# IRFM/librir

Measured on AMD Instinct MI355X. Metric: IR frames/sec encode+decode, 640x512 uint16, higher is better.
Workload: dtype u16; 1 GPU; configs[1]: 1000-frame 640x512 uint16 stream (S1 noisy background, seed 1234+rank), lossless RIRB1 encode+decode, device-resident, GOP 50, per GPU; two launches per step: the encoder leaves the PACKED form (headers + position and length per segment + the payload without holes: encoded_footprint_bytes, in a buffer of half the raw size), the decoder reads it as it is; the compressed payload (17 % of; frames_per_gpu=1000, width=640, height=512, gop=50

## Files before the change

librir_amd/csrc/codec_kernels.hip:

```cpp
#include <hip/hip_runtime.h>
#include <algorithm>
#include <stdint.h>

#include "codec_format.h"
#include "filter_kernels.h"
#include "runtime.h"

namespace rir
{

	constexpr int FRAME_LOAD_AUX = 2;
	constexpr int FRAME_STORE_AUX = 2;
	constexpr int SPARSE_STORE_AUX = 0;
	constexpr int STREAM_LOAD_AUX = 0;

	typedef short short2v __attribute__((ext_vector_type(2)));
	typedef unsigned short ushort2v __attribute__((ext_vector_type(2)));

	__device__ __forceinline__ uint32_t pk_sub16(uint32_t a, uint32_t b)
	{
		return __builtin_bit_cast(uint32_t, __builtin_bit_cast(ushort2v, a) - __builtin_bit_cast(ushort2v, b));
	}
	__device__ __forceinline__ uint32_t pk_add16(uint32_t a, uint32_t b)
	{
// ... 539 lines not shown
	{
		__shared__ uint32_t wave_tot[4];
		__shared__ uint32_t carry_s;
		const int c = blockIdx.x, tid = threadIdx.x, lane = tid & 63, wv = tid >> 6;
		const uint32_t *in = seg_words + (int64_t)c * ntiles;
		uint32_t *off = tile_off + (int64_t)c * (ntiles + 1);
		if (tid == 0)
			carry_s = 0;
		__syncthreads();
		for (int base = 0; base < ntiles; base += 256)
		{
			const int i = base + tid;
			const uint32_t v = i < ntiles ? in[i] : 0u;
			const uint32_t inc = wave_scan_add(v, lane);
			if (lane == 63)
				wave_tot[wv] = inc;
			__syncthreads();
			uint32_t pre = carry_s;
			for (int k = 0; k < wv; ++k)
				pre += wave_tot[k];
			if (i < ntiles)
				off[i] = pre + inc - v;
			__syncthreads();
			if (tid == 255)
				carry_s = pre + inc;
			__syncthreads();
		}
		if (tid == 0)
		{
			off[ntiles] = carry_s;
			chunk_words[c] = carry_s;
		}
	}

	__global__ __launch_bounds__(256) void rirb1_compact(const uint64_t *__restrict__ sparse, const uint32_t *__restrict__ tile_off,
														const uint64_t *__restrict__ chunk_words, int ntiles, int nchunks, int gop,
														uint64_t *__restrict__ chunk_off, uint64_t *__restrict__ stream)
	{
		const int t = blockIdx.x, c = blockIdx.y, tid = threadIdx.x;
		const uint32_t *off = tile_off + (int64_t)c * (ntiles + 1);
		const uint32_t o0 = off[t], o1 = off[t + 1];
		uint64_t s = 0;
		for (int i = tid & 63; i < c; i += 64)
			s += chunk_words[i];
#pragma unroll
		for (int d = 32; d >= 1; d >>= 1)
			s += (uint64_t)__shfl_xor((long long)s, d, 64);
		if (t == 0 && tid == 0)
		{
			chunk_off[c] = s;
			if (c == nchunks - 1)
				chunk_off[nchunks] = s + chunk_words[c];
		}
		const uint32_t n = o1 - o0;
		const uint64_t *src = sparse + ((int64_t)c * ntiles + t) * RIRB1_SLOT_WORDS(gop);
		uint64_t *dst = stream + s + o0;
		uint32_t i = tid;
		for (; i + 768 < n; i += 1024)
		{
			const uint64_t v0 = __builtin_nontemporal_load(src + i);
			const uint64_t v1 = __builtin_nontemporal_load(src + i + 256);
			const uint64_t v2 = __builtin_nontemporal_load(src + i + 512);
			const uint64_t v3 = __builtin_nontemporal_load(src + i + 768);
			dst[i] = v0, dst[i + 256] = v1, dst[i + 512] = v2, dst[i + 768] = v3;
		}
		for (; i < n; i += 256)
			dst[i] = __builtin_nontemporal_load(src + i);
	}

#define RIR_LB_TAG (1ull << 63)
#define RIR_LB_TIMEOUT_TICKS 200000000ull
	constexpr int LB_SLEEP = 8;
#define RIR_NONE 0xffffffffu

	struct RecordWords
	{
		v2u32 va, vb;
		uint32_t ia, ib;
	};

	__device__ __forceinline__ uint64_t emit_words_narrow(const Px8 &r, uint32_t mode, uint32_t base, RecordWords &rw, uint32_t pos, const LaneConsts &lc,
														  const TransposeConsts &tc, uint32_t *words)
	{
		uint32_t x = (r.d[0] | (r.d[1] << 8)) | ((r.d[2] | (r.d[3] << 8)) << 4);
		x = transpose32(x, tc);
		const uint64_t nz64 = __ballot(x != 0);
		const uint32_t nz = (uint32_t)nz64 | (uint32_t)(nz64 >> 32);
		uint32_t M = nz | ((nz >> 1) & 0x77777777u);
		M |= (M >> 2) & 0x33333333u;
		uint32_t W = M - ((M >> 1) & 0x55555555u);
		W = (W & 0x33333333u) + ((W >> 2) & 0x33333333u);
		*words = (uint32_t)__builtin_popcount(M);
		auto sw = __builtin_amdgcn_permlane32_swap(x, x, false, false);
		rw.va.x = x, rw.va.y = sw[1];
		rw.ia = __builtin_amdgcn_inverse_ballot_w64((uint64_t)M) ? pos + (uint32_t)__builtin_popcount(M & lc.p_before) : RIR_NONE;
		rw.vb = rw.va, rw.ib = RIR_NONE;
		const uint32_t B = base | (mode << 16);
		const uint64_t hw = __ballot((int32_t)(W << lc.p_hshw) < 0) & 0x00E700E700E700E7ull;
		const uint64_t hb = __ballot((int32_t)(B << lc.p_hshb) < 0) & 0x3C003C003C00FC00ull;
		return hw | hb;
	}

	__device__ __forceinline__ uint64_t emit_words_wide(const Px8 &r, uint32_t mode, uint32_t base, RecordWords &rw, uint32_t pos, const LaneConsts &lc,
														const TransposeConsts &tc, uint32_t *words)
	{
		uint32_t alo = r.d[0], ahi = r.d[1], blo = r.d[2], bhi = r.d[3];
		transpose64x2(alo, ahi, blo, bhi, tc);
		const uint32_t wa = row_allmax((alo | ahi) != 0 ? lc.bitp1 : 0u);
		const uint32_t wb = row_allmax((blo | bhi) != 0 ? lc.bitp1 : 0u);
		const uint32_t ia = rows_inclusive_sum(wa), ib = rows_inclusive_sum(wb);
		const uint32_t tot_a = (uint32_t)__builtin_amdgcn_readlane((int)ia, 63);
		const uint32_t tot_b = (uint32_t)__builtin_amdgcn_readlane((int)ib, 63);
		rw.va.x = alo, rw.va.y = ahi, rw.vb.x = blo, rw.vb.y = bhi;
		rw.ia = lc.bit < wa ? pos + ia - wa + lc.bit : RIR_NONE;
		rw.ib = lc.bit < wb ? pos + tot_a + ib - wb + lc.bit : RIR_NONE;
		*words = tot_a + tot_b;
		const uint32_t nib = (base >> lc.sh4) & 15u;
		const uint32_t field = ((nib << 10) | (lc.row0 ? mode << 14 : 0u)) | ((wb << 5) | wa);
		return __ballot((field & lc.onehot) != 0);
	}

	struct Staging
	{
		uint64_t *lds;
		uint32_t cap;
		uint32_t lds_used;
		bool spilling;
		__amdgpu_buffer_rsrc_t spill;
		uint64_t *arena;
		unsigned long long *cursor;
		uint64_t arena_words;
		uint32_t need;
		uint64_t extent;
		uint32_t *error_word;
	};

	__device__ __noinline__ uint64_t staging_take_extent(unsigned long long *cursor, uint32_t need, uint64_t arena_words, uint32_t *error_word)
	{
		unsigned long long off = 0;
		if ((threadIdx.x & 63u) == 0)
			off = __hip_atomic_fetch_add(cursor, (unsigned long long)need, __ATOMIC_RELAXED, __HIP_MEMORY_SCOPE_AGENT);
		const uint32_t lo = (uint32_t)__builtin_amdgcn_readfirstlane((int)(uint32_t)off);
		const uint32_t hi = (uint32_t)__builtin_amdgcn_readfirstlane((int)(uint32_t)(off >> 32));
		off = ((unsigned long long)hi << 32) | lo;
		if (off + need > arena_words)
		{
			if ((threadIdx.x & 63u) == 0)
				__hip_atomic_fetch_or(error_word, 2u, __ATOMIC_RELAXED, __HIP_MEMORY_SCOPE_AGENT);
			return ~0ull;
		}
		return off;
	}

	__device__ __forceinline__ uint64_t emit_staged(const Px8 &r, uint32_t mode, uint32_t base, Staging &sg, uint32_t pos, const LaneConsts &lc,
													const TransposeConsts &tc, uint32_t *words)
	{
		const uint32_t any = (r.d[0] | r.d[1]) | (r.d[2] | r.d[3]);
		RecordWords rw;
		uint64_t h;
		if (__ballot((any & 0xfff0fff0u) != 0) == 0)
			h = emit_words_narrow(r, mode, base, rw, pos, lc, tc, words);
		else
			h = emit_words_wide(r, mode, base, rw, pos, lc, tc, words);
		if (!sg.spilling && pos + *words > sg.cap)
		{
			sg.spilling = true, sg.lds_used = pos;
			if (sg.arena)
			{
				const uint64_t ext = staging_take_extent(sg.cursor, sg.need, sg.arena_words, sg.error_word);
				sg.extent = ((uint64_t)(uint32_t)__builtin_amdgcn_readfirstlane((int)(uint32_t)(ext >> 32)) << 32) |
							(uint32_t)__builtin_amdgcn_readfirstlane((int)(uint32_t)ext);
				if (sg.extent != ~0ull)
					sg.spill = make_rsrc(sg.arena + sg.extent, sg.need * 8u);
			}
		}
		if (!sg.spilling)
		{
			if (rw.ia != RIR_NONE)
				sg.lds[rw.ia] = ((uint64_t)rw.va.y << 32) | rw.va.x;
			if (rw.ib != RIR_NONE)
				sg.lds[rw.ib] = ((uint64_t)rw.vb.y << 32) | rw.vb.x;
		}
		const uint32_t add = sg.spilling ? 0u - sg.lds_used * 8u : RIR_OOB;
		const uint32_t oa = rw.ia != RIR_NONE ? rw.ia * 8u + add : RIR_OOB;
		const uint32_t ob = rw.ib != RIR_NONE ? rw.ib * 8u + add : RIR_OOB;
		__builtin_amdgcn_raw_buffer_store_b64(rw.va, sg.spill, oa, 0, SPARSE_STORE_AUX);
		__builtin_amdgcn_raw_buffer_store_b64(rw.vb, sg.spill, ob, 0, SPARSE_STORE_AUX);
		return h;
	}

	template <bool FAST>
	__device__ __forceinline__ uint32_t encode_run(const uint16_t *__restrict__ frames, int64_t npx, int nload, int64_t frame_first, bool has_key,
												   int tile, int lane, uint64_t *__restrict__ hdr_first, Staging &sg)
	{
		const int64_t p0 = (int64_t)tile * RIRB1_TILE_PX + lane * 8;
		const TransposeConsts tc = make_transpose_consts(lane);
		const LaneConsts lc = make_lane_consts(lane);
		const uint32_t lane_off = (uint32_t)lane * 16u;
		const uint16_t *next_ptr = frames + frame_first * npx + (int64_t)tile * RIRB1_TILE_PX;
		int next_f = 0;
		auto load = [&](int f, v4u32 &dst) {
			if (FAST)
			{
				const Px8 p = buf_load8(next_ptr, next_f < nload ? lane_off : RIR_OOB);
				dst.x = p.d[0], dst.y = p.d[1], dst.z = p.d[2], dst.w = p.d[3];
				next_ptr += npx;
				next_f += 1;
			}
			else
			{
				const Px8 p = load8(frames, frame_first + min(f, nload - 1), npx, p0, false);
				dst.x = p.d[0], dst.y = p.d[1], dst.z = p.d[2], dst.w = p.d[3];
			}
		};
		auto as_px8 = [](const v4u32 &v) {
			Px8 p;
			p.d[0] = v.x, p.d[1] = v.y, p.d[2] = v.z, p.d[3] = v.w;
			return p;
		};
		uint32_t pos = 0;
		uint64_t hdr_reg = 0;
		v4u32 s0, s1, s2, s3;
		load(0, s0);
		load(1, s1);
		load(2, s2);
		load(3, s3);
		if (has_key)
		{
			const Px8 cur = as_px8(s0);
			const uint32_t base_raw = tile_base(cur, false);
			const uint32_t b2 = base_raw | (base_raw << 16);
			Px8 r_raw;
#pragma unroll
			for (int k = 0; k < 4; ++k)
				r_raw.d[k] = pk_sub16(cur.d[k], b2);
			const Px8 dl = left_delta(cur, lane);
			const uint32_t base_left = tile_base(dl, true);
			const uint32_t bl2 = base_left | (base_left << 16);
			Px8 r_left;
#pragma unroll
			for (int k = 0; k < 4; ++k)
				r_left.d[k] = pk_sub16(dl.d[k], bl2);
			const bool use_left = payload_words(r_left) < payload_words(r_raw);
			Px8 r_sel;
#pragma unroll
			for (int k = 0; k < 4; ++k)
				r_sel.d[k] = use_left ? r_left.d[k] : r_raw.d[k];
			uint32_t words;
			const uint32_t key_mode = use_left ? RIRB1_MODE_LEFT : RIRB1_MODE_RAW;
			const uint64_t h = emit_staged(r_sel, key_mode, use_left ? base_left : base_raw, sg, pos, lc, tc, &words);
			if (lane == 0)
				hdr_first[0] = h;
			pos += words;
		}
#define RIR_ENC2_STEP(F, CUR, PREV)                                                            \
	{                                                                                          \
		const int f = (F);                                                                     \
		Px8 d;                                                                                 \
		{                                                                                      \
			const Px8 c_ = as_px8(CUR), p_ = as_px8(PREV);                                     \
			_Pragma("unroll") for (int k = 0; k < 4; ++k) d.d[k] = pk_sub16(c_.d[k], p_.d[k]); \
		}                                                                                      \
		load(f + 3, PREV);                                                                     \
		const uint32_t base = tile_base(d, true);                                              \
		const uint32_t b2 = base | (base << 16);                                               \
		_Pragma("unroll") for (int k = 0; k < 4; ++k) d.d[k] = pk_sub16(d.d[k], b2);          \
		uint32_t words;                                                                        \
		const uint64_t h = emit_staged(d, RIRB1_MODE_TEMPORAL, base, sg, pos, lc, tc, &words); \
		if (lane == ((f - 1) & 63))                                                            \
			hdr_reg = h;                                                                       \
		pos += words;                                                                          \
	}
		int fb = 1;
		while (fb < nload)
		{
			const int g0 = fb, gend = min(fb + 64, nload);
			for (; fb + 3 < gend; fb += 4)
			{
				RIR_ENC2_STEP(fb, s1, s0)
				RIR_ENC2_STEP(fb + 1, s2, s1)
				RIR_ENC2_STEP(fb + 2, s3, s2)
				RIR_ENC2_STEP(fb + 3, s0, s3)
			}
			if (fb < gend)
			{
				RIR_ENC2_STEP(fb, s1, s0)
				if (fb + 1 < gend)
				{
					RIR_ENC2_STEP(fb + 1, s2, s1)
					if (fb + 2 < gend)
						RIR_ENC2_STEP(fb + 2, s3, s2)
				}
				fb = gend;
			}
			if (g0 + lane < gend)
				hdr_first[g0 + lane] = hdr_reg;
			hdr_reg = 0;
		}
#undef RIR_ENC2_STEP
		return pos;
	}

	__device__ __forceinline__ uint64_t wave_sum_u64(uint64_t v)
	{
#pragma unroll
		for (int d = 32; d >= 1; d >>= 1)
			v += (uint64_t)__shfl_xor((long long)v, d, 64);
		return v;
	}

	__device__ __noinline__ bool encode_lookback(const uint64_t *P, const uint64_t *gtotal, const uint64_t *gran, uint32_t *error_word, int c, int t,
												 int ntiles, int ngroups, int lane, uint64_t *A_out, uint64_t *P_out, uint64_t * )
	{
		const int g = t >> 6, e1 = t & 63, E = e1 + g + (c > 0 ? 1 : 0);
		uint64_t accA = 0, accP = 0;
		const uint64_t t_start = __builtin_amdgcn_s_memrealtime();
		for (int e0 = 0; e0 < E; e0 += 64)
		{
			const int e = e0 + lane;
			const bool valid = e < E;
			int kind = 2;
			const uint64_t *ptr = P + c;
			if (e < e1)
				kind = 0, ptr = gran + (int64_t)c * ntiles + ((int64_t)g << 6) + e;
			else if (e < e1 + g)
				kind = 1, ptr = gtotal + (int64_t)c * ngroups + (e - e1);
			uint64_t v = 0;
			bool done = !valid;
			for (uint32_t spins = 0;; ++spins)
			{
				if (!done)
				{
					v = __hip_atomic_load(ptr, __ATOMIC_RELAXED, __HIP_MEMORY_SCOPE_AGENT);
					done = (v >> 63) != 0;
				}
				if (__ballot(!done) == 0)
					break;
				if ((spins & 15u) == 15u)
				{
					const uint32_t err = __hip_atomic_load(error_word, __ATOMIC_RELAXED, __HIP_MEMORY_SCOPE_AGENT);
					if (err != 0 || __builtin_amdgcn_s_memrealtime() - t_start > RIR_LB_TIMEOUT_TICKS)
					{
						if (lane == 0)
							__hip_atomic_store(error_word, 1u, __ATOMIC_RELAXED, __HIP_MEMORY_SCOPE_AGENT);
						return false;
					}
				}
				__builtin_amdgcn_s_sleep(LB_SLEEP);
			}
			if (valid)
			{
				if (kind == 2)
					accP = v & ~RIR_LB_TAG;
				else
					accA += v & ~RIR_LB_TAG;
			}
		}
		*A_out = wave_sum_u64(accA);
		*P_out = wave_sum_u64(accP);
		return true;
	}

	__device__ __host__ __forceinline__ int enc_split(int w, int waves, int nf)
	{
		if (w <= 0)
			return 0;
		if (w >= waves)
			return nf;
		const int b = (w * (nf + 1) + waves / 2) / waves - 1;
		return b < 1 ? (nf < 1 ? nf : 1) : (b > nf ? nf : b);
	}

	__device__ __host__ __forceinline__ int64_t enc_ctrl_words64(int nchunks, int ntiles)
	{
		const int64_t ngroups = (ntiles + 63) / 64;
		return 8 * 16 + 16 + ((int64_t)nchunks + 1) + (int64_t)nchunks * ngroups + (((int64_t)nchunks * ntiles + 15) & ~(int64_t)15) +
			   (int64_t)nchunks * ngroups + nchunks + 16;
	}

	template <int WAVES>
	__attribute__((amdgpu_waves_per_eu(8, 8))) __global__ __launch_bounds__(WAVES * 64) void rirb1_encode_dense(
		const uint16_t *__restrict__ frames, int64_t npx, int ntiles, int nframes, int gop, int nchunks, uint64_t *__restrict__ hdr_table,
		uint32_t *__restrict__ tile_off, uint64_t *__restrict__ chunk_off, uint64_t *__restrict__ stream, uint64_t *__restrict__ ctrl,
		uint64_t *__restrict__ spill, int cap)
	{
		extern __shared__ __attribute__((aligned(16))) uint64_t enc_lds[];
		uint64_t *sh_base = enc_lds + (size_t)WAVES * cap;
		uint32_t *sh_u32 = reinterpret_cast<uint32_t *>(sh_base + 1);
		const int lane = threadIdx.x & 63;
		const int w = __builtin_amdgcn_readfirstlane((int)(threadIdx.x >> 6));
		const int ngroups = (ntiles + 63) >> 6;
		uint32_t *heads = reinterpret_cast<uint32_t *>(ctrl);
		uint32_t *error_word = reinterpret_cast<uint32_t *>(ctrl + 8 * 16);
		uint64_t *P = ctrl + 8 * 16 + 16;
		uint64_t *gtotal = P + nchunks + 1;
		uint64_t *gran = gtotal + (int64_t)nchunks * ngroups;
		uint64_t *gcount = gran + (((int64_t)nchunks * ntiles + 15) & ~(int64_t)15);
		uint64_t *ccount = gcount + (int64_t)nchunks * ngroups;

		if (threadIdx.x == 0)
		{
			const uint32_t head = blockIdx.x & 7u;
			const uint32_t ticket = __hip_atomic_fetch_add(heads + head * 32, 1u, __ATOMIC_RELAXED, __HIP_MEMORY_SCOPE_AGENT);
			sh_u32[WAVES] = ticket * 8u + head;
		}
		__syncthreads();
		const int seg = __builtin_amdgcn_readfirstlane((int)sh_u32[WAVES]);
		const int chunk = seg / ntiles, tile = seg - chunk * ntiles;
		const int f_begin = chunk * gop;
		const int nf = min(gop, nframes - f_begin);
		uint64_t *my_hdr = hdr_table + (int64_t)seg * gop;

		const int rec0 = enc_split(w, WAVES, nf), rec1 = enc_split(w + 1, WAVES, nf);
		const int nrec = rec1 - rec0;
		const bool has_key = w == 0;
		const int first_load = has_key ? 0 : rec0 - 1;
		const int nload = nrec > 0 ? rec1 - first_load : 0;
		Staging sg;
		sg.lds = enc_lds + (size_t)w * cap;
		sg.cap = (uint32_t)cap;
		sg.lds_used = 0;
		sg.spilling = false;
		sg.arena = nullptr, sg.cursor = nullptr, sg.arena_words = 0, sg.need = 0, sg.extent = 0, sg.error_word = nullptr;
		uint64_t *my_spill = spill + (int64_t)seg * RIRB1_SLOT_WORDS(gop) + (int64_t)rec0 * RIRB1_REC_MAX_WORDS;
		sg.spill = make_rsrc(my_spill, (uint32_t)(nrec > 0 ? nrec : 0) * RIRB1_REC_MAX_WORDS * 8u);
		uint32_t pos = 0;
		if (nrec > 0)
		{
			const bool fast = ((npx & 7) == 0) && ((int64_t)(tile + 1) * RIRB1_TILE_PX <= npx) && ((((uintptr_t)frames) & 15) == 0);
			if (fast)
				pos = encode_run<true>(frames, npx, nload, (int64_t)f_begin + first_load, has_key, tile, lane, my_hdr + first_load, sg);
			else
				pos = encode_run<false>(frames, npx, nload, (int64_t)f_begin + first_load, has_key, tile, lane, my_hdr + first_load, sg);
		}
		for (int f = nf + (int)threadIdx.x; f < gop; f += WAVES * 64)
			my_hdr[f] = 0;
		if (lane == 0)
		{
			sh_u32[w] = pos;
			sh_u32[WAVES + 2 + w] = sg.spilling ? sg.lds_used : pos;
		}
		if (sg.spilling)
			asm volatile("s_waitcnt vmcnt(0)" ::: "memory");
		__syncthreads();
		if (w != 0)
			return;
		uint32_t total = 0;
#pragma unroll
		for (int i = 0; i < WAVES; ++i)
			total += sh_u32[i];
		bool chunk_last = false;
		uint64_t chunk_words = 0;
		if (lane == 0)
		{
			__hip_atomic_store(gran + (int64_t)chunk * ntiles + tile, RIR_LB_TAG | total, __ATOMIC_RELAXED, __HIP_MEMORY_SCOPE_AGENT);
			const int g = tile >> 6, gsize = min(64, ntiles - (g << 6));
			const uint64_t one = 1ull << 40, sum_mask = one - 1ull;
			const uint64_t og = __hip_atomic_fetch_add(gcount + (int64_t)chunk * ngroups + g, one | total, __ATOMIC_RELAXED, __HIP_MEMORY_SCOPE_AGENT);
			if ((int)(og >> 40) == gsize - 1)
			{
				const uint64_t gsum = (og & sum_mask) + total;
				__hip_atomic_store(gtotal + (int64_t)chunk * ngroups + g, RIR_LB_TAG | gsum, __ATOMIC_RELAXED, __HIP_MEMORY_SCOPE_AGENT);
				const uint64_t oc = __hip_atomic_fetch_add(ccount + chunk, one | gsum, __ATOMIC_RELAXED, __HIP_MEMORY_SCOPE_AGENT);
				if ((int)(oc >> 40) == ngroups - 1)
					chunk_last = true, chunk_words = (oc & sum_mask) + gsum;
			}
		}
		uint64_t A = 0, Pc = 0;
		const bool ok = encode_lookback(P, gtotal, gran, error_word, chunk, tile, ntiles, ngroups, lane, &A, &Pc, nullptr);
		if (!ok)
			return;
		if (lane == 0)
		{
			tile_off[(int64_t)chunk * (ntiles + 1) + tile] = (uint32_t)A;
			if (seg == 0)
				chunk_off[0] = 0;
			if (chunk_last)
			{
				tile_off[(int64_t)chunk * (ntiles + 1) + ntiles] = (uint32_t)chunk_words;
				__hip_atomic_store(P + chunk + 1, RIR_LB_TAG | (Pc + chunk_words), __ATOMIC_RELAXED, __HIP_MEMORY_SCOPE_AGENT);
				chunk_off[chunk + 1] = Pc + chunk_words;
			}
		}
		uint64_t *dst = stream + (Pc + A);
		for (int i = 0; i < WAVES; ++i)
		{
			const uint64_t *src = enc_lds + (size_t)i * cap;
			const uint32_t n_all = sh_u32[i], n_lds = sh_u32[WAVES + 2 + i];
			uint32_t j = (uint32_t)lane;
			for (; j + 192 < n_lds; j += 256)
			{
				const uint64_t v0 = src[j], v1 = src[j + 64], v2 = src[j + 128], v3 = src[j + 192];
				dst[j] = v0, dst[j + 64] = v1, dst[j + 128] = v2, dst[j + 192] = v3;
			}
			for (; j < n_lds; j += 64)
				dst[j] = src[j];
			if (n_all > n_lds)
			{
				const int r0 = enc_split(i, WAVES, nf), r1 = enc_split(i + 1, WAVES, nf);
				const __amdgpu_buffer_rsrc_t sp =
					make_rsrc(spill + (int64_t)seg * RIRB1_SLOT_WORDS(gop) + (int64_t)r0 * RIRB1_REC_MAX_WORDS, (uint32_t)(r1 - r0) * RIRB1_REC_MAX_WORDS * 8u);
				for (uint32_t q = (uint32_t)lane; q < n_all - n_lds; q += 64)
				{
					const v2u32 v = __builtin_amdgcn_raw_buffer_load_b64(sp, q * 8u, 0, 16 );
					dst[n_lds + q] = ((uint64_t)v.y << 32) | v.x;
				}
			}
			dst += n_all;
		}
	}

#define RIR_PACKED_COUNT_SHIFT 40
#define RIR_PACKED_WORDS_MASK ((1ull << RIR_PACKED_COUNT_SHIFT) - 1)
	__device__ __noinline__ void packed_finish(uint64_t *ctrl, uint64_t capacity_words, uint32_t sides)
	{
		if ((threadIdx.x & 63u) != 0)
			return;
		uint32_t *meet = reinterpret_cast<uint32_t *>(ctrl + 80);
		if (sides > 1 && __hip_atomic_fetch_add(meet, 1u, __ATOMIC_RELAXED, __HIP_MEMORY_SCOPE_AGENT) + 1 < sides)
			return;
		unsigned long long *c = reinterpret_cast<unsigned long long *>(ctrl);
		const uint64_t low = __hip_atomic_exchange(c, 0ull, __ATOMIC_RELAXED, __HIP_MEMORY_SCOPE_AGENT) & RIR_PACKED_WORDS_MASK;
		const uint64_t high = __hip_atomic_exchange(c + 16, 0ull, __ATOMIC_RELAXED, __HIP_MEMORY_SCOPE_AGENT) & RIR_PACKED_WORDS_MASK;
		const uint64_t spill = __hip_atomic_exchange(c + 32, 0ull, __ATOMIC_RELAXED, __HIP_MEMORY_SCOPE_AGENT);
		const uint32_t err = __hip_atomic_exchange(reinterpret_cast<uint32_t *>(ctrl + 48), 0u, __ATOMIC_RELAXED, __HIP_MEMORY_SCOPE_AGENT);
		__hip_atomic_store(meet, 0u, __ATOMIC_RELAXED, __HIP_MEMORY_SCOPE_AGENT);
		ctrl[64] = low, ctrl[65] = high, ctrl[66] = spill, ctrl[67] = err, ctrl[68] = capacity_words;
	}
	template <int WAVES, bool FAST>
	__attribute__((amdgpu_waves_per_eu(8, 8))) __global__ __launch_bounds__(WAVES * 64) void rirb1_encode_packed(
		const uint16_t *__restrict__ frames, int64_t npx, int ntiles, int tile_first, int nframes, int gop, uint64_t *__restrict__ hdr_table,
		uint64_t *__restrict__ seg_pos, uint32_t *__restrict__ seg_words, uint64_t *__restrict__ stream, uint64_t capacity_words,
		uint64_t *__restrict__ ctrl, uint64_t *__restrict__ arena, uint64_t arena_words, int cap, int diag)
	{
		extern __shared__ __attribute__((aligned(16))) uint64_t enc_lds[];
		uint64_t *sh_u64 = enc_lds + (size_t)WAVES * cap;
		uint32_t *sh_u32 = reinterpret_cast<uint32_t *>(sh_u64 + 1 + WAVES);
		const int lane = threadIdx.x & 63;
		const int w = __builtin_amdgcn_readfirstlane((int)(threadIdx.x >> 6));
		const int chunk = blockIdx.y, tile = tile_first + blockIdx.x;
		const bool downwards = ((tile + chunk) & 1) != 0 && diag != 1;
		unsigned long long *cursor = reinterpret_cast<unsigned long long *>(ctrl) + (downwards ? 16 : 0);
		unsigned long long *spill_cursor = reinterpret_cast<unsigned long long *>(ctrl + 32);
		uint32_t *error_word = reinterpret_cast<uint32_t *>(ctrl + 48);

		const int64_t seg = (int64_t)chunk * ntiles + tile;
		const int f_begin = chunk * gop;
		const int nf = min(gop, nframes - f_begin);
		uint64_t *my_hdr = hdr_table + seg * gop;

		const int rec0 = enc_split(w, WAVES, nf), rec1 = enc_split(w + 1, WAVES, nf);
		const int nrec = rec1 - rec0;
		const bool has_key = w == 0;
		const int first_load = has_key ? 0 : rec0 - 1;
		const int nload = nrec > 0 ? rec1 - first_load : 0;
		Staging sg;
		sg.lds = enc_lds + (size_t)w * cap;
		sg.cap = (uint32_t)cap;
		sg.lds_used = 0;
		sg.spilling = false;
		sg.spill = make_rsrc(arena, 0);
		sg.arena = arena, sg.cursor = spill_cursor, sg.arena_words = arena_words, sg.error_word = error_word;
		sg.need = (uint32_t)(nrec > 0 ? nrec : 0) * RIRB1_REC_MAX_WORDS;
		sg.extent = ~0ull;
		uint32_t pos = 0;
		if (nrec > 0)
			pos = encode_run<FAST>(frames, npx, nload, (int64_t)f_begin + first_load, has_key, tile, lane, my_hdr + first_load, sg);
		for (int f = nf + (int)threadIdx.x; f < gop; f += WAVES * 64)
			my_hdr[f] = 0;
		if (lane == 0)
		{
			sh_u32[w] = pos;
			sh_u32[WAVES + w] = sg.spilling ? sg.lds_used : pos;
			sh_u64[1 + w] = sg.extent;
		}
		if (sg.spilling)
			asm volatile("s_waitcnt vmcnt(0)" ::: "memory");
		__syncthreads();
		if (w != 0)
			return;
		uint32_t total = 0;
		bool lost = false;
#pragma unroll
		for (int i = 0; i < WAVES; ++i)
		{
			const uint32_t n = sh_u32[i];
			total += n;
			lost |= n > sh_u32[WAVES + i] && sh_u64[1 + i] == ~0ull;
		}
		if (w == 0)
		{
			unsigned long long at = 0;
			if (lane == 0)
				at = __hip_atomic_fetch_add(cursor, (unsigned long long)total | (1ull << RIR_PACKED_COUNT_SHIFT), __ATOMIC_RELAXED,
											__HIP_MEMORY_SCOPE_AGENT);
			const uint32_t lo = (uint32_t)__builtin_amdgcn_readfirstlane((int)(uint32_t)at);
			const uint32_t hi = (uint32_t)__builtin_amdgcn_readfirstlane((int)(uint32_t)(at >> 32));
			const uint32_t arrived = hi >> (RIR_PACKED_COUNT_SHIFT - 32);
			const uint64_t nseg = (uint64_t)gridDim.y * (uint32_t)ntiles;
			const uint64_t on_side = diag == 1 ? nseg : downwards ? nseg / 2 : (nseg + 1) / 2;
			if ((uint64_t)arrived + 1 == on_side)
				packed_finish(ctrl, capacity_words, diag == 1 || nseg < 2 ? 1u : 2u);
			at = ((unsigned long long)hi << 32 | lo) & RIR_PACKED_WORDS_MASK;
			const bool fits = at + total <= capacity_words;
			if (downwards)
				at = capacity_words - at - total;
			if (lane == 0)
			{
				seg_pos[seg] = at;
				seg_words[seg] = total;
				sh_u64[0] = (fits && !lost) ? at : ~0ull;
			}
			if (!fits || lost)
				return;
			uint64_t *dst = stream + at;
			for (int i = 0; i < WAVES; ++i)
			{
				const uint64_t *src = enc_lds + (size_t)i * cap;
				const uint32_t n_all = sh_u32[i], n_lds = sh_u32[WAVES + i];
				uint32_t j = (uint32_t)lane;
				for (; j + 192 < n_lds; j += 256)
				{
					const uint64_t v0 = src[j], v1 = src[j + 64], v2 = src[j + 128], v3 = src[j + 192];
					dst[j] = v0, dst[j + 64] = v1, dst[j + 128] = v2, dst[j + 192] = v3;
				}
				for (; j < n_lds; j += 64)
					dst[j] = src[j];
				if (n_all > n_lds)
				{
					const int r0 = enc_split(i, WAVES, nf), r1 = enc_split(i + 1, WAVES, nf);
					const __amdgpu_buffer_rsrc_t sp = make_rsrc(arena + sh_u64[1 + i], (uint32_t)(r1 - r0) * RIRB1_REC_MAX_WORDS * 8u);
					for (uint32_t q = (uint32_t)lane; q < n_all - n_lds; q += 64)
					{
						const v2u32 v = __builtin_amdgcn_raw_buffer_load_b64(sp, q * 8u, 0, 16 );
						dst[n_lds + q] = ((uint64_t)v.y << 32) | v.x;
					}
				}
				dst += n_all;
			}
		}
	}

	struct Fetched
	{
		uint64_t hdr;
		v2u32 a, b;
		uint32_t words;
		bool bad;
		bool narrow;
	};

	__device__ __forceinline__ bool header_is_narrow(uint64_t hdr)
	{
		const uint64_t m0 = 0x0021002100210021ull;
		const uint64_t hi = hdr & (m0 * 0x18u);
		const uint64_t b2 = (hdr >> 2) & m0;
		const uint64_t lo = (hdr | (hdr >> 1)) & m0;
		return (hi | (b2 & lo)) == 0;
	}

	__device__ __forceinline__ Fetched fetch_record(uint64_t hdr, __amdgpu_buffer_rsrc_t in, uint32_t pos, uint32_t seg_len, const LaneConsts &lc)
	{
		Fetched r;
		r.hdr = hdr;
		r.narrow = header_is_narrow(hdr);
		const bool hdr_bad = ((hdr & 0xC000C000C0000000ull) != 0) || (((hdr >> 14) & 3u) == 3u);
		uint32_t oa, ob;
		if (r.narrow)
		{
			const uint32_t w = ((lc.n_hhi ? (uint32_t)(hdr >> 32) : (uint32_t)hdr) >> lc.n_hsh) & 31u;
			const uint32_t incl = half_inclusive_sum(lc.n_first ? w : 0u);
			r.words = (uint32_t)__builtin_amdgcn_readlane((int)incl, 31);
			r.bad = hdr_bad || (pos + r.words > seg_len);
			oa = (!r.bad && lc.n_half == 0 && lc.n_bit < w) ? (pos + incl - w + lc.n_bit) * 8u : RIR_OOB;
			ob = RIR_OOB;
		}
		else
		{
			const uint32_t field = ((lc.row_hi ? (uint32_t)(hdr >> 32) : (uint32_t)hdr) >> lc.sh16) & 0xffffu;
			const uint32_t wa = field & 31u, wb = (field >> 5) & 31u;
			const uint32_t ia = rows_inclusive_sum(wa), ib = rows_inclusive_sum(wb);
			const uint32_t tot_a = (uint32_t)__builtin_amdgcn_readlane((int)ia, 63);
			const uint32_t tot_b = (uint32_t)__builtin_amdgcn_readlane((int)ib, 63);
			r.words = tot_a + tot_b;
			const bool too_wide = __ballot(wa > 16u || wb > 16u) != 0;
			r.bad = hdr_bad || too_wide || (pos + r.words > seg_len);
			oa = (!r.bad && lc.bit < wa) ? (pos + ia - wa + lc.bit) * 8u : RIR_OOB;
			ob = (!r.bad && lc.bit < wb) ? (pos + tot_a + ib - wb + lc.bit) * 8u : RIR_OOB;
		}
		r.a = __builtin_amdgcn_raw_buffer_load_b64(in, oa, 0, STREAM_LOAD_AUX);
		r.b = __builtin_amdgcn_raw_buffer_load_b64(in, ob, 0, STREAM_LOAD_AUX);
		return r;
	}

	__device__ __forceinline__ Px8 planes_to_residuals(v2u32 a, v2u32 b, bool narrow, const TransposeConsts &tc)
	{
		Px8 r;
		if (narrow)
		{
			auto sw = __builtin_amdgcn_permlane32_swap(a.x, a.y, false, false);
			const uint32_t x = transpose32(sw[0], tc);
			const uint32_t lo = x & 0x0f0f0f0fu, hi = (x >> 4) & 0x0f0f0f0fu;
			r.d[0] = __builtin_amdgcn_perm(hi, lo, 0x0c040c00u);
			r.d[1] = __builtin_amdgcn_perm(hi, lo, 0x0c050c01u);
			r.d[2] = __builtin_amdgcn_perm(hi, lo, 0x0c060c02u);
			r.d[3] = __builtin_amdgcn_perm(hi, lo, 0x0c070c03u);
		}
		else
		{
			uint32_t alo = a.x, ahi = a.y, blo = b.x, bhi = b.y;
			transpose64x2(alo, ahi, blo, bhi, tc);
			r.d[0] = alo, r.d[1] = ahi, r.d[2] = blo, r.d[3] = bhi;
		}
		return r;
	}

	__device__ __forceinline__ uint64_t readlane64(uint64_t v, int l)
	{
		return (uint64_t)(uint32_t)__builtin_amdgcn_readlane((int)(uint32_t)v, l) |
			   ((uint64_t)(uint32_t)__builtin_amdgcn_readlane((int)(uint32_t)(v >> 32), l) << 32);
	}

	__device__ __forceinline__ Px8 left_integrate(const Px8 &d, int lane)
	{
		uint32_t a[8];
#pragma unroll
		for (int k = 0; k < 4; ++k)
		{
			a[2 * k] = d.d[k] & 0xffffu;
			a[2 * k + 1] = d.d[k] >> 16;
		}
#pragma unroll
		for (int i = 1; i < 8; ++i)
			a[i] = (a[i] + a[i - 1]) & 0xffffu;
		const uint32_t incl = wave_scan_add(a[7], lane);
		const uint32_t carry = (incl - a[7]) & 0xffffu;
		Px8 o;
#pragma unroll
		for (int k = 0; k < 4; ++k)
			o.d[k] = ((a[2 * k] + carry) & 0xffffu) | (((a[2 * k + 1] + carry) & 0xffffu) << 16);
		return o;
	}

	struct ChunkSink
	{
		uint16_t *frames, *tile0;
		int64_t npx, frame0, p0;
		uint32_t lane_off;
		__device__ __forceinline__ ChunkSink(uint16_t *frames_, int64_t npx_, int64_t frame0_, int tile, int lane)
			: frames(frames_), tile0(frames_ + frame0_ * npx_ + (int64_t)tile * RIRB1_TILE_PX), npx(npx_), frame0(frame0_),
			  p0((int64_t)tile * RIRB1_TILE_PX + lane * 8), lane_off((uint32_t)lane * 16u)
		{
		}
		template <bool FAST>
		__device__ __forceinline__ void put(int f, const Px8 &o)
		{
			if (FAST)
				buf_store8(tile0 + (int64_t)f * npx, lane_off, o);
			else
				store8(frames, frame0 + f, npx, p0, false, o);
		}
	};

	template <bool FAST, class Sink>
	__device__ __forceinline__ void decode_tile(const uint64_t *__restrict__ my_hdr, const uint64_t *__restrict__ in_ptr, uint32_t seg_len,
												int nf, bool check_end, int lane, Sink &sink, int *__restrict__ error_flag)
	{
		const TransposeConsts tc = make_transpose_consts(lane);
		const LaneConsts lc = make_lane_consts(lane);
		const __amdgpu_buffer_rsrc_t in = make_rsrc(in_ptr, seg_len * 8u);

		Px8 prev;
		prev.d[0] = prev.d[1] = prev.d[2] = prev.d[3] = 0;
		uint32_t pos = 0;
		bool err = false;
		for (int f0 = 0; f0 < nf; f0 += 64)
		{
			const int nr = min(64, nf - f0);
			const uint64_t my_h = lane < nr ? my_hdr[f0 + lane] : 0ull;
			Fetched r0 = fetch_record(readlane64(my_h, 0), in, pos, seg_len, lc);
			pos += r0.words;
			Fetched r1 = fetch_record(nr > 1 ? readlane64(my_h, 1) : 0ull, in, pos, seg_len, lc);
			pos += r1.words;
			Fetched r2 = fetch_record(nr > 2 ? readlane64(my_h, 2) : 0ull, in, pos, seg_len, lc);
			pos += r2.words;
			Fetched r3 = fetch_record(nr > 3 ? readlane64(my_h, 3) : 0ull, in, pos, seg_len, lc);
			pos += r3.words;
#define RIR_DEC_STEP(FR, R)                                                                                          \
// ... 388 lines not shown
```

Before: 3.773 million frames/s.

## Version encode loop into LDS-only hot path and spill cold path

Splits the encoder's per-record staging into a hot loop that only writes to LDS and records the first record that would overflow capacity. On overflow it takes a spill extent, replays from that frame, and finishes in a cold loop that writes every record to the global spill arena. This removes the per-step spill checks and the predicated buffer stores from the common path, at the cost of larger code and reloading frames after an overflow.

Result: faster. 3.811 million frames/s, median of 6 (+1.0%).

```diff
diff --git a/librir_amd/csrc/codec_kernels.hip b/librir_amd/csrc/codec_kernels.hip
--- a/librir_amd/csrc/codec_kernels.hip
+++ b/librir_amd/csrc/codec_kernels.hip
@@ -715,44 +715,82 @@
 		return off;
 	}
 
-	__device__ __forceinline__ uint64_t emit_staged(const Px8 &r, uint32_t mode, uint32_t base, Staging &sg, uint32_t pos, const LaneConsts &lc,
-													const TransposeConsts &tc, uint32_t *words)
-	{
-		const uint32_t any = (r.d[0] | r.d[1]) | (r.d[2] | r.d[3]);
-		RecordWords rw;
-		uint64_t h;
-		if (__ballot((any & 0xfff0fff0u) != 0) == 0)
-			h = emit_words_narrow(r, mode, base, rw, pos, lc, tc, words);
-		else
-			h = emit_words_wide(r, mode, base, rw, pos, lc, tc, words);
-		if (!sg.spilling && pos + *words > sg.cap)
-		{
-			sg.spilling = true, sg.lds_used = pos;
-			if (sg.arena)
-			{
-				const uint64_t ext = staging_take_extent(sg.cursor, sg.need, sg.arena_words, sg.error_word);
-				sg.extent = ((uint64_t)(uint32_t)__builtin_amdgcn_readfirstlane((int)(uint32_t)(ext >> 32)) << 32) |
-							(uint32_t)__builtin_amdgcn_readfirstlane((int)(uint32_t)ext);
-				if (sg.extent != ~0ull)
-					sg.spill = make_rsrc(sg.arena + sg.extent, sg.need * 8u);
-			}
-		}
-		if (!sg.spilling)
-		{
-			if (rw.ia != RIR_NONE)
-				sg.lds[rw.ia] = ((uint64_t)rw.va.y << 32) | rw.va.x;
-			if (rw.ib != RIR_NONE)
-				sg.lds[rw.ib] = ((uint64_t)rw.vb.y << 32) | rw.vb.x;
-		}
-		const uint32_t add = sg.spilling ? 0u - sg.lds_used * 8u : RIR_OOB;
+	__device__ __forceinline__ void staging_begin_spill(Staging &sg, uint32_t pos)
+	{
+		sg.spilling = true, sg.lds_used = pos;
+		if (sg.arena)
+		{
+			const uint64_t ext = staging_take_extent(sg.cursor, sg.need, sg.arena_words, sg.error_word);
+			sg.extent = ((uint64_t)(uint32_t)__builtin_amdgcn_readfirstlane((int)(uint32_t)(ext >> 32)) << 32) |
+						(uint32_t)__builtin_amdgcn_readfirstlane((int)(uint32_t)ext);
+			if (sg.extent != ~0ull)
+				sg.spill = make_rsrc(sg.arena + sg.extent, sg.need * 8u);
+		}
+	}
+	__device__ __forceinline__ void staging_put_lds(const Staging &sg, const RecordWords &rw)
+	{
+		if (rw.ia != RIR_NONE)
+			sg.lds[rw.ia] = ((uint64_t)rw.va.y << 32) | rw.va.x;
+		if (rw.ib != RIR_NONE)
+			sg.lds[rw.ib] = ((uint64_t)rw.vb.y << 32) | rw.vb.x;
+	}
+	__device__ __forceinline__ void staging_put_spill(const Staging &sg, const RecordWords &rw, uint32_t add)
+	{
 		const uint32_t oa = rw.ia != RIR_NONE ? rw.ia * 8u + add : RIR_OOB;
 		const uint32_t ob = rw.ib != RIR_NONE ? rw.ib * 8u + add : RIR_OOB;
 		__builtin_amdgcn_raw_buffer_store_b64(rw.va, sg.spill, oa, 0, SPARSE_STORE_AUX);
 		__builtin_amdgcn_raw_buffer_store_b64(rw.vb, sg.spill, ob, 0, SPARSE_STORE_AUX);
+	}
+	__device__ __forceinline__ uint64_t emit_words(const Px8 &r, uint32_t mode, uint32_t base, RecordWords &rw, uint32_t pos, const LaneConsts &lc,
+												   const TransposeConsts &tc, uint32_t *words)
+	{
+		const uint32_t any = (r.d[0] | r.d[1]) | (r.d[2] | r.d[3]);
+		if (__ballot((any & 0xfff0fff0u) != 0) == 0)
+			return emit_words_narrow(r, mode, base, rw, pos, lc, tc, words);
+		return emit_words_wide(r, mode, base, rw, pos, lc, tc, words);
+	}
+
+	template <bool SPILLED>
+	__device__ __forceinline__ uint64_t emit_staged(const Px8 &r, uint32_t mode, uint32_t base, Staging &sg, uint32_t pos, const LaneConsts &lc,
+													const TransposeConsts &tc, uint32_t *words)
+	{
+		RecordWords rw;
+		const uint64_t h = emit_words(r, mode, base, rw, pos, lc, tc, words);
+		if (!SPILLED)
+		{
+			if (!sg.spilling && pos + *words > sg.cap)
+				staging_begin_spill(sg, pos);
+			if (!sg.spilling)
+				staging_put_lds(sg, rw);
+		}
+		staging_put_spill(sg, rw, SPILLED || sg.spilling ? 0u - sg.lds_used * 8u : RIR_OOB);
 		return h;
 	}
 
-	template <bool FAST>
+	__device__ __forceinline__ void key_residuals(const Px8 &cur, int lane, Px8 &r_sel, uint32_t &mode, uint32_t &base)
+	{
+		const uint32_t base_raw = tile_base(cur, false);
+		const uint32_t b2 = base_raw | (base_raw << 16);
+		Px8 r_raw;
+#pragma unroll
+		for (int k = 0; k < 4; ++k)
+			r_raw.d[k] = pk_sub16(cur.d[k], b2);
+		const Px8 dl = left_delta(cur, lane);
+		const uint32_t base_left = tile_base(dl, true);
+		const uint32_t bl2 = base_left | (base_left << 16);
+		Px8 r_left;
+#pragma unroll
+		for (int k = 0; k < 4; ++k)
+			r_left.d[k] = pk_sub16(dl.d[k], bl2);
+		const bool use_left = payload_words(r_left) < payload_words(r_raw);
+#pragma unroll
+		for (int k = 0; k < 4; ++k)
+			r_sel.d[k] = use_left ? r_left.d[k] : r_raw.d[k];
+		mode = use_left ? RIRB1_MODE_LEFT : RIRB1_MODE_RAW;
+		base = use_left ? base_left : base_raw;
+	}
+
+	template <bool FAST, bool VERSIONED>
 	__device__ __forceinline__ uint32_t encode_run(const uint16_t *__restrict__ frames, int64_t npx, int nload, int64_t frame_first, bool has_key,
 												   int tile, int lane, uint64_t *__restrict__ hdr_first, Staging &sg)
 	{
@@ -783,6 +821,13 @@
 		};
 		uint32_t pos = 0;
 		uint64_t hdr_reg = 0;
+		int fb = 1;
+		RecordWords ow;
+		uint64_t oh = 0;
+		uint32_t owords = 0;
+		int of = 0;
+		uint32_t over = 0;
+		ow.va.x = ow.va.y = ow.vb.x = ow.vb.y = 0, ow.ia = ow.ib = RIR_NONE;
 		v4u32 s0, s1, s2, s3;
 		load(0, s0);
 		load(1, s1);
@@ -790,34 +835,29 @@
 		load(3, s3);
 		if (has_key)
 		{
-			const Px8 cur = as_px8(s0);
-			const uint32_t base_raw = tile_base(cur, false);
-			const uint32_t b2 = base_raw | (base_raw << 16);
-			Px8 r_raw;
-#pragma unroll
-			for (int k = 0; k < 4; ++k)
-				r_raw.d[k] = pk_sub16(cur.d[k], b2);
-			const Px8 dl = left_delta(cur, lane);
-			const uint32_t base_left = tile_base(dl, true);
-			const uint32_t bl2 = base_left | (base_left << 16);
-			Px8 r_left;
-#pragma unroll
-			for (int k = 0; k < 4; ++k)
-				r_left.d[k] = pk_sub16(dl.d[k], bl2);
-			const bool use_left = payload_words(r_left) < payload_words(r_raw);
 			Px8 r_sel;
-#pragma unroll
-			for (int k = 0; k < 4; ++k)
-				r_sel.d[k] = use_left ? r_left.d[k] : r_raw.d[k];
-			uint32_t words;
-			const uint32_t key_mode = use_left ? RIRB1_MODE_LEFT : RIRB1_MODE_RAW;
-			const uint64_t h = emit_staged(r_sel, key_mode, use_left ? base_left : base_raw, sg, pos, lc, tc, &words);
-			if (lane == 0)
-				hdr_first[0] = h;
-			pos += words;
-		}
-#define RIR_ENC2_STEP(F, CUR, PREV)                                                            \
-	{                                                                                          \
+			uint32_t key_mode, key_base, words;
+			uint64_t h;
+			key_residuals(as_px8(s0), lane, r_sel, key_mode, key_base);
+			if (VERSIONED)
+			{
+				RecordWords rw;
+				h = emit_words(r_sel, key_mode, key_base, rw, pos, lc, tc, &words);
+				if (pos + words > sg.cap)
+					ow = rw, oh = h, owords = words, of = 0, over = 1;
+				else
+					staging_put_lds(sg, rw);
+			}
+			else
+				h = emit_staged<false>(r_sel, key_mode, key_base, sg, pos, lc, tc, &words);
+			if (!over)
+			{
+				if (lane == 0)
+					hdr_first[0] = h;
+				pos += words;
+			}
+		}
+#define RIR_ENC2_DELTA(F, CUR, PREV)                                                           \
 		const int f = (F);                                                                     \
 		Px8 d;                                                                                 \
 		{                                                                                      \
@@ -828,39 +868,151 @@
 		const uint32_t base = tile_base(d, true);                                              \
 		const uint32_t b2 = base | (base << 16);                                               \
 		_Pragma("unroll") for (int k = 0; k < 4; ++k) d.d[k] = pk_sub16(d.d[k], b2);          \
-		uint32_t words;                                                                        \
-		const uint64_t h = emit_staged(d, RIRB1_MODE_TEMPORAL, base, sg, pos, lc, tc, &words); \
+		uint32_t words;
+#define RIR_ENC2_HOT_STEP(F, CUR, PREV)                                                        \
+	{                                                                                          \
+		RIR_ENC2_DELTA(F, CUR, PREV)                                                           \
+		RecordWords rw;                                                                        \
+		const uint64_t h = emit_words(d, RIRB1_MODE_TEMPORAL, base, rw, pos, lc, tc, &words);  \
+		if (!over)                                                                             \
+		{                                                                                      \
+			if (pos + words > sg.cap)                                                          \
+				ow = rw, oh = h, owords = words, of = f, over = 1;                             \
+			else                                                                               \
+			{                                                                                  \
+				staging_put_lds(sg, rw);                                                       \
+				if (lane == ((f - 1) & 63))                                                    \
+					hdr_reg = h;                                                               \
+				pos += words;                                                                  \
+			}                                                                                  \
+		}                                                                                      \
+		asm volatile("" : "+s"(over));                                                         \
+	}
+#define RIR_ENC2_STEP(F, CUR, PREV)                                                            \
+	{                                                                                          \
+		RIR_ENC2_DELTA(F, CUR, PREV)                                                           \
+		const uint64_t h = emit_staged<VERSIONED>(d, RIRB1_MODE_TEMPORAL, base, sg, pos, lc, tc, &words); \
 		if (lane == ((f - 1) & 63))                                                            \
 			hdr_reg = h;                                                                       \
 		pos += words;                                                                          \
 	}
-		int fb = 1;
-		while (fb < nload)
-		{
-			const int g0 = fb, gend = min(fb + 64, nload);
-			for (; fb + 3 < gend; fb += 4)
-			{
-				RIR_ENC2_STEP(fb, s1, s0)
-				RIR_ENC2_STEP(fb + 1, s2, s1)
-				RIR_ENC2_STEP(fb + 2, s3, s2)
-				RIR_ENC2_STEP(fb + 3, s0, s3)
-			}
-			if (fb < gend)
-			{
-				RIR_ENC2_STEP(fb, s1, s0)
-				if (fb + 1 < gend)
+		if (!VERSIONED)
+		{
+			while (fb < nload)
+			{
+				const int g0 = fb, gend = min(fb + 64, nload);
+				for (; fb + 3 < gend; fb += 4)
 				{
+					RIR_ENC2_STEP(fb, s1, s0)
 					RIR_ENC2_STEP(fb + 1, s2, s1)
-					if (fb + 2 < gend)
-						RIR_ENC2_STEP(fb + 2, s3, s2)
+					RIR_ENC2_STEP(fb + 2, s3, s2)
+					RIR_ENC2_STEP(fb + 3, s0, s3)
 				}
-				fb = gend;
-			}
-			if (g0 + lane < gend)
+				if (fb < gend)
+				{
+					RIR_ENC2_STEP(fb, s1, s0)
+					if (fb + 1 < gend)
+					{
+						RIR_ENC2_STEP(fb + 1, s2, s1)
+						if (fb + 2 < gend)
+							RIR_ENC2_STEP(fb + 2, s3, s2)
+					}
+					fb = gend;
+				}
+				if (g0 + lane < gend)
+					hdr_first[g0 + lane] = hdr_reg;
+				hdr_reg = 0;
+			}
+			return pos;
+		}
+		while (fb + 3 < nload && !over)
+		{
+			const int gend = min(fb + 64, nload);
+			while (fb + 3 < gend && !over)
+			{
+				RIR_ENC2_HOT_STEP(fb, s1, s0)
+				RIR_ENC2_HOT_STEP(fb + 1, s2, s1)
+				RIR_ENC2_HOT_STEP(fb + 2, s3, s2)
+				RIR_ENC2_HOT_STEP(fb + 3, s0, s3)
+				fb += 4;
+			}
+			if (!over && ((fb - 1) & 63) == 0)
+			{
+				hdr_first[fb - 64 + lane] = hdr_reg;
+				hdr_reg = 0;
+			}
+		}
+		if (!over && fb < nload)
+		{
+			RIR_ENC2_HOT_STEP(fb, s1, s0)
+			if (fb + 1 < nload)
+			{
+				RIR_ENC2_HOT_STEP(fb + 1, s2, s1)
+				if (fb + 2 < nload)
+					RIR_ENC2_HOT_STEP(fb + 2, s3, s2)
+			}
+		}
+		if (!over)
+		{
+			if (((nload - 1) & 63) != 0)
+			{
+				const int g0 = ((nload - 2) & ~63) + 1;
+				if (g0 + lane < nload)
+					hdr_first[g0 + lane] = hdr_reg;
+			}
+			return pos;
+		}
+		staging_begin_spill(sg, pos);
+		staging_put_spill(sg, ow, 0u - sg.lds_used * 8u);
+		pos += owords;
+		next_ptr = frames + (frame_first + of) * npx + (int64_t)tile * RIRB1_TILE_PX;
+		next_f = of;
+		load(of, s0);
+		load(of + 1, s1);
+		load(of + 2, s2);
+		load(of + 3, s3);
+		if (of == 0)
+		{
+			if (lane == 0)
+				hdr_first[0] = oh;
+		}
+		else
+		{
+			if (lane == ((of - 1) & 63))
+				hdr_reg = oh;
+			if ((of & 63) == 0)
+				hdr_first[of - 63 + lane] = hdr_reg, hdr_reg = 0;
+		}
+#define RIR_ENC2_COLD_STEP(F, CUR, PREV)                                                       \
+	{                                                                                          \
+		RIR_ENC2_STEP(F, CUR, PREV)                                                            \
+		if (((F) & 63) == 0)                                                                   \
+			hdr_first[(F) - 63 + lane] = hdr_reg, hdr_reg = 0;                                 \
+	}
+		for (fb = of + 1; fb < nload; fb += 4)
+		{
+			RIR_ENC2_COLD_STEP(fb, s1, s0)
+			if (fb + 1 < nload)
+			{
+				RIR_ENC2_COLD_STEP(fb + 1, s2, s1)
+				if (fb + 2 < nload)
+				{
+					RIR_ENC2_COLD_STEP(fb + 2, s3, s2)
+					if (fb + 3 < nload)
+						RIR_ENC2_COLD_STEP(fb + 3, s0, s3)
+				}
+			}
+		}
+		if (((nload - 1) & 63) != 0)
+		{
+			const int g0 = ((nload - 2) & ~63) + 1;
+			if (g0 + lane < nload)
 				hdr_first[g0 + lane] = hdr_reg;
-			hdr_reg = 0;
-		}
+		}
+#undef RIR_ENC2_COLD_STEP
 #undef RIR_ENC2_STEP
+#undef RIR_ENC2_HOT_STEP
+#undef RIR_ENC2_DELTA
 		return pos;
 	}
 
@@ -992,9 +1144,9 @@
 		{
 			const bool fast = ((npx & 7) == 0) && ((int64_t)(tile + 1) * RIRB1_TILE_PX <= npx) && ((((uintptr_t)frames) & 15) == 0);
 			if (fast)
-				pos = encode_run<true>(frames, npx, nload, (int64_t)f_begin + first_load, has_key, tile, lane, my_hdr + first_load, sg);
+				pos = encode_run<true, false>(frames, npx, nload, (int64_t)f_begin + first_load, has_key, tile, lane, my_hdr + first_load, sg);
 			else
-				pos = encode_run<false>(frames, npx, nload, (int64_t)f_begin + first_load, has_key, tile, lane, my_hdr + first_load, sg);
+				pos = encode_run<false, false>(frames, npx, nload, (int64_t)f_begin + first_load, has_key, tile, lane, my_hdr + first_load, sg);
 		}
 		for (int f = nf + (int)threadIdx.x; f < gop; f += WAVES * 64)
 			my_hdr[f] = 0;
@@ -1128,7 +1280,7 @@
 		sg.extent = ~0ull;
 		uint32_t pos = 0;
 		if (nrec > 0)
-			pos = encode_run<FAST>(frames, npx, nload, (int64_t)f_begin + first_load, has_key, tile, lane, my_hdr + first_load, sg);
+			pos = encode_run<FAST, true>(frames, npx, nload, (int64_t)f_begin + first_load, has_key, tile, lane, my_hdr + first_load, sg);
 		for (int f = nf + (int)threadIdx.x; f < gop; f += WAVES * 64)
 			my_hdr[f] = 0;
 		if (lane == 0)
```

## Encode even waves backward through their frame range with mirrored LDS staging

Applied to the files above, without the earlier changes.

Even-numbered waves in the encoder now walk their frame range in reverse, loading frames from the end. They place records at the top of their LDS staging area, and at the end of their spill extent when they overflow. The split between waves is mirrored so that adjacent waves share boundary frames, apparently to improve cache reuse of frame loads across waves. The copy-out loop is adjusted so the packed stream keeps record order. This adds index arithmetic and extra template instantiations, and the byte layout relies on the wave record ordering staying consistent.

After: 3.785 million frames/s before, 3.841 million frames/s after, median of 6. +1.5%, better.

```diff
diff --git a/librir_amd/csrc/codec_kernels.hip b/librir_amd/csrc/codec_kernels.hip
--- a/librir_amd/csrc/codec_kernels.hip
+++ b/librir_amd/csrc/codec_kernels.hip
@@ -715,16 +715,18 @@
 		return off;
 	}
 
+	template <int DIR>
 	__device__ __forceinline__ uint64_t emit_staged(const Px8 &r, uint32_t mode, uint32_t base, Staging &sg, uint32_t pos, const LaneConsts &lc,
 													const TransposeConsts &tc, uint32_t *words)
 	{
 		const uint32_t any = (r.d[0] | r.d[1]) | (r.d[2] | r.d[3]);
 		RecordWords rw;
 		uint64_t h;
+		const uint32_t rel = DIR > 0 ? pos : 0u;
 		if (__ballot((any & 0xfff0fff0u) != 0) == 0)
-			h = emit_words_narrow(r, mode, base, rw, pos, lc, tc, words);
+			h = emit_words_narrow(r, mode, base, rw, rel, lc, tc, words);
 		else
-			h = emit_words_wide(r, mode, base, rw, pos, lc, tc, words);
+			h = emit_words_wide(r, mode, base, rw, rel, lc, tc, words);
 		if (!sg.spilling && pos + *words > sg.cap)
 		{
 			sg.spilling = true, sg.lds_used = pos;
@@ -739,12 +741,13 @@
 		}
 		if (!sg.spilling)
 		{
+			uint64_t *rec = DIR > 0 ? sg.lds : sg.lds + (sg.cap - pos - *words);
 			if (rw.ia != RIR_NONE)
-				sg.lds[rw.ia] = ((uint64_t)rw.va.y << 32) | rw.va.x;
+				rec[rw.ia] = ((uint64_t)rw.va.y << 32) | rw.va.x;
 			if (rw.ib != RIR_NONE)
-				sg.lds[rw.ib] = ((uint64_t)rw.vb.y << 32) | rw.vb.x;
-		}
-		const uint32_t add = sg.spilling ? 0u - sg.lds_used * 8u : RIR_OOB;
+				rec[rw.ib] = ((uint64_t)rw.vb.y << 32) | rw.vb.x;
+		}
+		const uint32_t add = !sg.spilling ? RIR_OOB : DIR > 0 ? 0u - sg.lds_used * 8u : (sg.need - (pos - sg.lds_used) - *words) * 8u;
 		const uint32_t oa = rw.ia != RIR_NONE ? rw.ia * 8u + add : RIR_OOB;
 		const uint32_t ob = rw.ib != RIR_NONE ? rw.ib * 8u + add : RIR_OOB;
 		__builtin_amdgcn_raw_buffer_store_b64(rw.va, sg.spill, oa, 0, SPARSE_STORE_AUX);
@@ -752,27 +755,29 @@
 		return h;
 	}
 
-	template <bool FAST>
+	template <bool FAST, int DIR>
 	__device__ __forceinline__ uint32_t encode_run(const uint16_t *__restrict__ frames, int64_t npx, int nload, int64_t frame_first, bool has_key,
 												   int tile, int lane, uint64_t *__restrict__ hdr_first, Staging &sg)
 	{
+		constexpr bool BACK = DIR < 0;
 		const int64_t p0 = (int64_t)tile * RIRB1_TILE_PX + lane * 8;
 		const TransposeConsts tc = make_transpose_consts(lane);
 		const LaneConsts lc = make_lane_consts(lane);
 		const uint32_t lane_off = (uint32_t)lane * 16u;
-		const uint16_t *next_ptr = frames + frame_first * npx + (int64_t)tile * RIRB1_TILE_PX;
+		const uint16_t *next_ptr = frames + (frame_first + (BACK ? nload - 1 : 0)) * npx + (int64_t)tile * RIRB1_TILE_PX;
 		int next_f = 0;
-		auto load = [&](int f, v4u32 &dst) {
+		auto load = [&](int k, v4u32 &dst) {
 			if (FAST)
 			{
 				const Px8 p = buf_load8(next_ptr, next_f < nload ? lane_off : RIR_OOB);
 				dst.x = p.d[0], dst.y = p.d[1], dst.z = p.d[2], dst.w = p.d[3];
-				next_ptr += npx;
+				next_ptr = BACK ? next_ptr - npx : next_ptr + npx;
 				next_f += 1;
 			}
 			else
 			{
-				const Px8 p = load8(frames, frame_first + min(f, nload - 1), npx, p0, false);
+				const int i = min(k, nload - 1);
+				const Px8 p = load8(frames, frame_first + (BACK ? nload - 1 - i : i), npx, p0, false);
 				dst.x = p.d[0], dst.y = p.d[1], dst.z = p.d[2], dst.w = p.d[3];
 			}
 		};
@@ -783,14 +788,7 @@
 		};
 		uint32_t pos = 0;
 		uint64_t hdr_reg = 0;
-		v4u32 s0, s1, s2, s3;
-		load(0, s0);
-		load(1, s1);
-		load(2, s2);
-		load(3, s3);
-		if (has_key)
-		{
-			const Px8 cur = as_px8(s0);
+		auto key_record = [&](const Px8 &cur) {
 			const uint32_t base_raw = tile_base(cur, false);
 			const uint32_t b2 = base_raw | (base_raw << 16);
 			Px8 r_raw;
@@ -811,26 +809,33 @@
 				r_sel.d[k] = use_left ? r_left.d[k] : r_raw.d[k];
 			uint32_t words;
 			const uint32_t key_mode = use_left ? RIRB1_MODE_LEFT : RIRB1_MODE_RAW;
-			const uint64_t h = emit_staged(r_sel, key_mode, use_left ? base_left : base_raw, sg, pos, lc, tc, &words);
+			const uint64_t h = emit_staged<DIR>(r_sel, key_mode, use_left ? base_left : base_raw, sg, pos, lc, tc, &words);
 			if (lane == 0)
 				hdr_first[0] = h;
 			pos += words;
-		}
-#define RIR_ENC2_STEP(F, CUR, PREV)                                                            \
+		};
+		v4u32 s0, s1, s2, s3;
+		load(0, s0);
+		load(1, s1);
+		load(2, s2);
+		load(3, s3);
+		if (!BACK && has_key)
+			key_record(as_px8(s0));
+#define RIR_ENC2_STEP(K, NEW, OLD)                                                            \
 	{                                                                                          \
-		const int f = (F);                                                                     \
+		const int k_ = (K);                                                                    \
 		Px8 d;                                                                                 \
 		{                                                                                      \
-			const Px8 c_ = as_px8(CUR), p_ = as_px8(PREV);                                     \
+			const Px8 c_ = as_px8(BACK ? OLD : NEW), p_ = as_px8(BACK ? NEW : OLD);            \
 			_Pragma("unroll") for (int k = 0; k < 4; ++k) d.d[k] = pk_sub16(c_.d[k], p_.d[k]); \
 		}                                                                                      \
-		load(f + 3, PREV);                                                                     \
+		load(k_ + 3, OLD);                                                                     \
 		const uint32_t base = tile_base(d, true);                                              \
 		const uint32_t b2 = base | (base << 16);                                               \
 		_Pragma("unroll") for (int k = 0; k < 4; ++k) d.d[k] = pk_sub16(d.d[k], b2);          \
 		uint32_t words;                                                                        \
-		const uint64_t h = emit_staged(d, RIRB1_MODE_TEMPORAL, base, sg, pos, lc, tc, &words); \
-		if (lane == ((f - 1) & 63))                                                            \
+		const uint64_t h = emit_staged<DIR>(d, RIRB1_MODE_TEMPORAL, base, sg, pos, lc, tc, &words); \
+		if (lane == ((k_ - 1) & 63))                                                           \
 			hdr_reg = h;                                                                       \
 		pos += words;                                                                          \
 	}
@@ -857,10 +862,16 @@
 				fb = gend;
 			}
 			if (g0 + lane < gend)
-				hdr_first[g0 + lane] = hdr_reg;
+				hdr_first[BACK ? nload - (g0 + lane) : g0 + lane] = hdr_reg;
 			hdr_reg = 0;
 		}
 #undef RIR_ENC2_STEP
+		if (BACK && has_key)
+		{
+			const int ks = (nload - 1) & 3;
+			const v4u32 kv = ks == 0 ? s0 : ks == 1 ? s1 : ks == 2 ? s2 : s3;
+			key_record(as_px8(kv));
+		}
 		return pos;
 	}
 
@@ -934,6 +945,17 @@
 		return b < 1 ? (nf < 1 ? nf : 1) : (b > nf ? nf : b);
 	}
 
+	__device__ __host__ __forceinline__ bool enc_walks_back(int w) { return (w & 1) == 0; }
+	__device__ __host__ __forceinline__ int enc_split_mirrored(int w, int waves, int nf)
+	{
+		if (waves == 4 && w == 3)
+		{
+			const int c = 2 * enc_split(2, waves, nf) - enc_split(1, waves, nf);
+			return c > nf ? nf : c;
+		}
+		return enc_split(w, waves, nf);
+	}
+
 	__device__ __host__ __forceinline__ int64_t enc_ctrl_words64(int nchunks, int ntiles)
 	{
 		const int64_t ngroups = (ntiles + 63) / 64;
@@ -992,9 +1014,9 @@
 		{
 			const bool fast = ((npx & 7) == 0) && ((int64_t)(tile + 1) * RIRB1_TILE_PX <= npx) && ((((uintptr_t)frames) & 15) == 0);
 			if (fast)
-				pos = encode_run<true>(frames, npx, nload, (int64_t)f_begin + first_load, has_key, tile, lane, my_hdr + first_load, sg);
+				pos = encode_run<true, 1>(frames, npx, nload, (int64_t)f_begin + first_load, has_key, tile, lane, my_hdr + first_load, sg);
 			else
-				pos = encode_run<false>(frames, npx, nload, (int64_t)f_begin + first_load, has_key, tile, lane, my_hdr + first_load, sg);
+				pos = encode_run<false, 1>(frames, npx, nload, (int64_t)f_begin + first_load, has_key, tile, lane, my_hdr + first_load, sg);
 		}
 		for (int f = nf + (int)threadIdx.x; f < gop; f += WAVES * 64)
 			my_hdr[f] = 0;
@@ -1112,7 +1134,7 @@
 		const int nf = min(gop, nframes - f_begin);
 		uint64_t *my_hdr = hdr_table + seg * gop;
 
-		const int rec0 = enc_split(w, WAVES, nf), rec1 = enc_split(w + 1, WAVES, nf);
+		const int rec0 = enc_split_mirrored(w, WAVES, nf), rec1 = enc_split_mirrored(w + 1, WAVES, nf);
 		const int nrec = rec1 - rec0;
 		const bool has_key = w == 0;
 		const int first_load = has_key ? 0 : rec0 - 1;
@@ -1128,7 +1150,12 @@
 		sg.extent = ~0ull;
 		uint32_t pos = 0;
 		if (nrec > 0)
-			pos = encode_run<FAST>(frames, npx, nload, (int64_t)f_begin + first_load, has_key, tile, lane, my_hdr + first_load, sg);
+		{
+			if (enc_walks_back(w))
+				pos = encode_run<FAST, -1>(frames, npx, nload, (int64_t)f_begin + first_load, has_key, tile, lane, my_hdr + first_load, sg);
+			else
+				pos = encode_run<FAST, 1>(frames, npx, nload, (int64_t)f_begin + first_load, has_key, tile, lane, my_hdr + first_load, sg);
+		}
 		for (int f = nf + (int)threadIdx.x; f < gop; f += WAVES * 64)
 			my_hdr[f] = 0;
 		if (lane == 0)
@@ -1179,24 +1206,29 @@
 			uint64_t *dst = stream + at;
 			for (int i = 0; i < WAVES; ++i)
 			{
-				const uint64_t *src = enc_lds + (size_t)i * cap;
-				const uint32_t n_all = sh_u32[i], n_lds = sh_u32[WAVES + i];
+				const bool back = enc_walks_back(i);
+				const uint32_t n_all = sh_u32[i], n_lds = sh_u32[WAVES + i], n_ext = n_all - n_lds;
+				const uint64_t *src = enc_lds + (size_t)i * cap + (back ? (uint32_t)cap - n_lds : 0u);
+				uint64_t *dst_lds = dst + (back ? n_ext : 0u);
 				uint32_t j = (uint32_t)lane;
 				for (; j + 192 < n_lds; j += 256)
 				{
 					const uint64_t v0 = src[j], v1 = src[j + 64], v2 = src[j + 128], v3 = src[j + 192];
-					dst[j] = v0, dst[j + 64] = v1, dst[j + 128] = v2, dst[j + 192] = v3;
+					dst_lds[j] = v0, dst_lds[j + 64] = v1, dst_lds[j + 128] = v2, dst_lds[j + 192] = v3;
 				}
 				for (; j < n_lds; j += 64)
-					dst[j] = src[j];
-				if (n_all > n_lds)
+					dst_lds[j] = src[j];
+				if (n_ext > 0)
 				{
-					const int r0 = enc_split(i, WAVES, nf), r1 = enc_split(i + 1, WAVES, nf);
-					const __amdgpu_buffer_rsrc_t sp = make_rsrc(arena + sh_u64[1 + i], (uint32_t)(r1 - r0) * RIRB1_REC_MAX_WORDS * 8u);
-					for (uint32_t q = (uint32_t)lane; q < n_all - n_lds; q += 64)
+					const int r0 = enc_split_mirrored(i, WAVES, nf), r1 = enc_split_mirrored(i + 1, WAVES, nf);
+					const uint32_t need = (uint32_t)(r1 - r0) * RIRB1_REC_MAX_WORDS;
+					const __amdgpu_buffer_rsrc_t sp = make_rsrc(arena + sh_u64[1 + i], need * 8u);
+					const uint32_t first = back ? need - n_ext : 0u;
+					uint64_t *dst_ext = dst + (back ? 0u : n_lds);
+					for (uint32_t q = (uint32_t)lane; q < n_ext; q += 64)
 					{
-						const v2u32 v = __builtin_amdgcn_raw_buffer_load_b64(sp, q * 8u, 0, 16 );
-						dst[n_lds + q] = ((uint64_t)v.y << 32) | v.x;
+						const v2u32 v = __builtin_amdgcn_raw_buffer_load_b64(sp, (first + q) * 8u, 0, 16 );
+						dst_ext[q] = ((uint64_t)v.y << 32) | v.x;
 					}
 				}
 				dst += n_all;
```
